# arpg/Kangaroo

Hardware: AMD Instinct MI355X
Metric: kinectfusion_frames_per_sec_640x480_to_512cubed_tsdf (higher is better)
Workload: dtype f32

## Files before the change

### include/kfx_extras.h

```cpp
#ifndef KFX_EXTRAS_H
#define KFX_EXTRAS_H

#include "kfx.h"

#ifdef __cplusplus
extern "C" {
#endif

int kfx_bilateral_guided_f32(const kfx_image* out, const kfx_image* in, const kfx_image* guide, float gs, float gr, float gc,
                             unsigned size, kfx_stream stream);
int kfx_bilateral_guided_u8(const kfx_image* out, const kfx_image* in, const kfx_image* guide, float gs, float gr, float gc,
                            unsigned size, kfx_stream stream);

int kfx_disp2depth(const kfx_image* in, const kfx_image* out, float fu, float baseline, float min_disp, kfx_stream stream);
int kfx_filter_bad_kinect_f32(const kfx_image* out, const kfx_image* in, kfx_stream stream);
int kfx_filter_bad_kinect_u16(const kfx_image* out, const kfx_image* in, kfx_stream stream);
int kfx_colour_vbo(const kfx_image* id, const kfx_image* vbo, const kfx_image* rgb, const float KT_cd[12], kfx_stream stream);

typedef struct kfx_keyframe {
    float K[4];
    float T_iw[12];
    kfx_image img;
} kfx_keyframe;
int kfx_texture_depth(const kfx_image* img, const kfx_keyframe* kfs, int n_kf, const kfx_image* depth, const kfx_image* norm,
                      const kfx_image* phong, const float T_wd[12], const float Kdepth[4], kfx_stream stream);

int kfx_raycast_box(const kfx_image* imgd, const float T_wc[12], const float K[4], const float boxmin[3], const float boxmax[3],
                    kfx_stream stream);
int kfx_raycast_sphere(const kfx_image* imgd, const kfx_image* img, const float T_wc[12], const float K[4], const float center[3],
                       float r, kfx_stream stream);
int kfx_raycast_plane(const kfx_image* imgd, const kfx_image* img, const float T_wc[12], const float K[4], const float n_w[3],
                      kfx_stream stream);
int kfx_sdf_distance(const kfx_image* dist, const kfx_image* depth, const kfx_volume* vol, const float T_wc[12], const float K[4],
                     float trunc_distance, kfx_stream stream);

#ifdef __cplusplus
}
#endif
#endif
```

### kangaroo_amd/_lib.py

```python
import ctypes as C
import os

_HERE = os.path.dirname(os.path.abspath(__file__))
LIB_PATH = os.environ.get("KFX_LIB_PATH") or os.path.join(_HERE, "libkfx.so")


class KfxImage(C.Structure):
    _fields_ = [("pitch", C.c_size_t), ("ptr", C.c_void_p), ("w", C.c_size_t), ("h", C.c_size_t)]


class KfxVolume(C.Structure):
    _fields_ = [("pitch", C.c_size_t), ("ptr", C.c_void_p), ("w", C.c_size_t), ("h", C.c_size_t),
                ("img_pitch", C.c_size_t), ("d", C.c_size_t),
                ("boxmin", C.c_float * 3), ("boxmax", C.c_float * 3)]


class KfxLss6(C.Structure):
    _fields_ = [("JTy", C.c_float * 6), ("JTJ", C.c_float * 21), ("sqErr", C.c_float), ("obs", C.c_uint)]


class KfxIcpLevel(C.Structure):
    _fields_ = [("Pl", KfxImage), ("Pr", KfxImage), ("Nr", KfxImage), ("K", C.c_float * 4), ("iterations", C.c_int), ("rotation_only", C.c_int)]


# ... 47 lines not shown
    "kfx_sdf_sphere": (C.c_int, [PV, PF, C.c_float, C.c_void_p]),
    "kfx_raycast_sdf_slab": (C.c_int, [C.c_void_p, C.c_int, PV, C.POINTER(KfxSlab), C.c_int, C.c_int, C.c_int, C.c_int, PF, PF,
                                       C.c_float, C.c_float, C.c_float, C.c_int, C.c_void_p]),
    "kfx_raycast_sdf_slab_h": (C.c_int, [C.c_void_p, C.c_int, PV, C.POINTER(KfxSlab), C.c_int, C.c_int, C.c_int, C.c_int, PF, PF,
                                       C.c_float, C.c_float, C.c_float, C.c_int, C.c_void_p]),
    "kfx_raycast_sdf_slab_tiles": (C.c_int, [C.c_void_p, C.c_void_p, C.c_size_t, C.c_int, C.c_int, C.c_int, C.c_int, C.c_void_p, C.c_int, C.c_void_p, C.c_void_p, C.c_int,
                                             PV, C.POINTER(KfxSlab), C.c_int, C.c_int, C.c_int, C.c_int, PF, PF, C.c_float, C.c_float, C.c_float, C.c_int, C.c_void_p]),
    "kfx_raycast_state_to_images": (C.c_int, [PI, PI, PI, C.c_void_p, C.c_void_p]),
    "kfx_sdf_fuse_color": (C.c_int, [PV, PV, PI, PI, PF, PF, PI, PF, PF, C.c_float, C.c_float, C.c_float, C.c_uint, C.c_void_p]),
    "kfx_raycast_sdf_color": (C.c_int, [PI, PI, PI, PV, PV, PF, PF, C.c_float, C.c_float, C.c_float, C.c_int, C.c_void_p]),
    "kfx_color_reset": (C.c_int, [PV, C.c_void_p]),
    "kfx_sdf_fuse_color_tracked": (C.c_int, [PV, PV, C.c_void_p, PI, PI, PF, PF, PI, PF, PF, C.c_float, C.c_float, C.c_float, C.c_uint, C.c_void_p]),
    "kfx_raycast_color_hits": (C.c_int, [C.c_int, C.POINTER(PI), C.POINTER(PI), PV, PF, PF, C.c_void_p]),
    "kfx_sdf_fuse_color_slab": (C.c_int, [PV, PV, C.POINTER(KfxSlab), PI, PI, PF, PF, PI, PF, PF, C.c_float, C.c_float, C.c_float, C.c_uint, C.c_void_p]),
    "kfx_raycast_sdf_slab_color": (C.c_int, [C.c_void_p, C.c_int, PV, PV, C.POINTER(KfxSlab), C.c_int, C.c_int, C.c_int, C.c_int, PF, PF,
                                             C.c_float, C.c_float, C.c_float, C.c_int, C.c_void_p]),
    "kfx_raycast_sdf_slab_tiles_color": (C.c_int, [C.c_void_p, C.c_void_p, C.c_size_t, C.c_int, C.c_int, C.c_int, C.c_int, C.c_void_p, C.c_int, C.c_void_p, C.c_void_p,
                                                   C.c_int, PV, PV, C.POINTER(KfxSlab), C.c_int, C.c_int, C.c_int, C.c_int, PF, PF, C.c_float, C.c_float, C.c_float,
                                                   C.c_int, C.c_void_p]),
    "kfx_slab_raycast_exact_tiled_color": (C.c_int, [PI, PI, PI, C.c_void_p, PV, PV, C.c_void_p, PF, PF, C.c_float, C.c_float, C.c_float, C.c_int, C.c_int,
                                                     C.c_void_p, C.c_void_p, C.POINTER(C.c_int), C.POINTER(C.c_int)]),
    "kfx_slab_frame_set_color": (C.c_int, [C.c_void_p, PV, PI, PF, PF]),
    "kfx_depth_to_vbo_normals_f32": (C.c_int, [PI, PI, PI, PF, C.c_float, C.c_void_p]),
    "kfx_depth_pyramid_vbo_normals_f32": (C.c_int, [PI, PI, PI, PF, C.c_int, C.c_float, C.c_void_p]),
    "kfx_bilateral_guided_f32": (C.c_int, [PI, PI, PI, C.c_float, C.c_float, C.c_float, C.c_uint, C.c_void_p]),
    "kfx_bilateral_guided_u8": (C.c_int, [PI, PI, PI, C.c_float, C.c_float, C.c_float, C.c_uint, C.c_void_p]),
    "kfx_texture_depth": (C.c_int, [PI, C.POINTER(KfxKeyframe), C.c_int, PI, PI, PI, PF, PF, C.c_void_p]),
    "kfx_disp2depth": (C.c_int, [PI, PI, C.c_float, C.c_float, C.c_float, C.c_void_p]),
    "kfx_filter_bad_kinect_f32": (C.c_int, [PI, PI, C.c_void_p]),
    "kfx_filter_bad_kinect_u16": (C.c_int, [PI, PI, C.c_void_p]),
    "kfx_colour_vbo": (C.c_int, [PI, PI, PI, PF, C.c_void_p]),
    "kfx_raycast_box": (C.c_int, [PI, PF, PF, PF, PF, C.c_void_p]),
    "kfx_raycast_sphere": (C.c_int, [PI, PI, PF, PF, PF, C.c_float, C.c_void_p]),
    "kfx_raycast_plane": (C.c_int, [PI, PI, PF, PF, PF, C.c_void_p]),
    "kfx_sdf_distance": (C.c_int, [PI, PI, PV, PF, PF, C.c_float, C.c_void_p]),
    "kfx_mc_count": (C.c_int, [PV, C.c_void_p, C.c_void_p]),
    "kfx_mc_emit": (C.c_int, [PV, PV, C.c_void_p, C.c_void_p, C.c_longlong, C.c_void_p, C.c_void_p, C.c_void_p, C.c_void_p]),
    "kfx_mesh_scratch_bytes": (C.c_size_t, [PV, C.c_int, C.POINTER(KfxSlab), C.c_int, C.c_int]),
    "kfx_mesh_plan": (C.c_int, [PV, C.c_int, C.POINTER(KfxSlab), C.c_int, C.c_int, C.c_void_p, C.c_size_t, C.POINTER(C.c_ulonglong), C.c_void_p]),
    "kfx_mesh_emit": (C.c_int, [PV, C.c_int, C.POINTER(KfxSlab), C.c_int, C.c_int, PV, C.c_void_p, C.c_size_t, C.POINTER(C.c_ulonglong), C.c_void_p,
                                C.c_void_p, C.c_void_p, C.c_void_p, C.c_void_p, C.c_void_p]),
    "kfx_icp_refine": (C.c_int, [C.POINTER(KfxIcpLevel), C.c_int, C.c_float, C.c_float, PI, PI, C.POINTER(C.c_double), PF,
                                 C.POINTER(C.c_uint), C.POINTER(C.c_int), C.c_void_p]),
    "kfx_pose_step": (C.c_int, [C.POINTER(C.c_double), C.POINTER(C.c_double), C.POINTER(C.c_double), PF]),
    "kfx_icp_refine_then": (C.c_int, [C.POINTER(KfxIcpLevel), C.c_int, C.c_float, C.c_float, PI, PI, C.POINTER(C.c_double), PF,
                                      C.POINTER(C.c_uint), C.POINTER(C.c_int), C.c_void_p, C.c_void_p, C.c_void_p]),
# ... 85 lines not shown
```

### kangaroo_amd/csrc/frame.hip

```cpp
#include <cmath>
#include <cstdlib>
#include <new>

#include "kfx_device.h"

struct kfx_frame {
    kfx_frame_config cfg;
    kfx_sdf_summary* summary;
    int track;
    long long frames;
    int slots;
    hipEvent_t* ev;
    long long* ev_frame;
    unsigned char* ev_mask;
    unsigned mask;
    kfx_image texels;
};

using namespace kfx;

static int valid_image(const kfx_image& im, size_t elem)
{
    return im.ptr && im.w > 0 && im.h > 0 && im.pitch >= im.w * elem;
}
// ... 128 lines not shown
    if (f->slots && f->mask) {
        const int slot = (int)(f->frames % f->slots);
        ev = f->ev + (size_t)slot * 4;
        m = f->mask;
        f->ev_frame[slot] = f->frames;
        f->ev_mask[slot] = (unsigned char)m;
    } else if (f->slots) {
        f->ev_frame[(int)(f->frames % f->slots)] = -1;
    }
    const hipStream_t s = (hipStream_t)stream;
    int e = 0;
    const auto record = [&](int k) {
        if (!(m & (1u << k))) return;
        const hipError_t he = hipEventRecord(ev[k], s);
        if (he != hipSuccess) {
            (void)hipGetLastError();
            f->ev_mask[(int)(f->frames % f->slots)] &= (unsigned char)~(1u << k);
            if (!e) e = set_error((int)he, "kfx_frame_step: hipEventRecord");
        }
    };
    record(0);
    const kfx_image* tex = ((parts & KFX_FRAME_PREPROCESS) && (parts & KFX_FRAME_FUSE) && f->texels.ptr) ? &f->texels : nullptr;
    if (!e && (parts & KFX_FRAME_PREPROCESS)) {
        e = kfx_bilateral_f32(&c.filtered, src, c.bilateral_gs, c.bilateral_gr, c.bilateral_size, c.bilateral_minval, 1, stream);
        if (!e) e = depth_to_vbo_normals_texels(&c.vbo, &c.normals, &c.filtered, c.K, 1.0f, tex, stream);
    }
    record(1);
    if (!e && (parts & KFX_FRAME_FUSE))
        e = sdf_fuse_texels(&c.vol, f->track ? f->summary : nullptr, &c.filtered, &c.normals, tex, T_cw, c.K, c.trunc_dist, c.max_w, c.mincostheta, c.fuse_flags, stream);
    record(2);
    if (!e && (parts & KFX_FRAME_RAYCAST)) {
        if (f->track) e = kfx_raycast_sdf_tracked(&c.ray_depth, &c.ray_norm, &c.ray_img, &c.vol, f->summary, T_wc, c.K, c.near, c.far, c.trunc_dist, 1, stream);
        else e = kfx_raycast_sdf(&c.ray_depth, &c.ray_norm, &c.ray_img, &c.vol, T_wc, c.K, c.near, c.far, c.trunc_dist, 1, stream);
    }
    record(3);
    f->frames += 1;
    return e;
}

extern "C" int kfx_frame_timings(kfx_frame* f, long long first_frame, int n_frames, float* ms)
{
    if (!f || !ms) return set_error(KFX_E_NULL, "kfx_frame_timings: null argument");
    if (!f->slots) return set_error(KFX_E_RANGE, "kfx_frame_timings: the frame was created without timing slots");
    if (n_frames <= 0) return 0;
    const long long last = first_frame + n_frames - 1;
    if (first_frame < 0 || last >= f->frames || f->frames - first_frame > f->slots) return set_error(KFX_E_RANGE, "kfx_frame_timings: frames not in the ring");
    const auto slot_of = [&](long long fr) { return (int)(fr % f->slots); };
    const auto first_event = [](unsigned m) { for (int k = 0; k < 4; ++k) if (m & (1u << k)) return k; return -1; };
// ... 43 lines not shown
```

### kangaroo_amd/csrc/preprocess.hip

```cpp

#include "kfx_device.h"
#include "host_args.h"

namespace kfx {

constexpr int BIL_MAX_R = 16;

struct BilParams {
    const unsigned char* in;
    size_t in_pitch;
    unsigned char* out;
    size_t out_pitch;
    int w, h;
    int iw, ih;
    int R;
    float gs, gr;
    float minval;
    int use_minval;
};

template <typename Ti>
__device__ __forceinline__ float load_clamped(const BilParams& p, int x, int y)
{
    x = min(max(x, 0), p.iw - 1);
    y = min(max(y, 0), p.ih - 1);
    return (float)reinterpret_cast<const Ti*>(p.in + (size_t)y * p.in_pitch)[x];
}

template <typename Ti, int TX, int TY, int PY>
__global__ __launch_bounds__(TX * TY) void k_bilateral(const BilParams p)
{
    extern __shared__ __attribute__((aligned(16))) float lds[];
    constexpr int NT = TX * TY;
    const int R = p.R, D = 2 * R + 1;
    const int TW = TX + 2 * R, TH = TY * PY + 2 * R;
    float* tile = lds;
    float* sw = lds + TW * TH;
    const int tid = threadIdx.x;
    const int bx = blockIdx.x * TX, by = blockIdx.y * (TY * PY);

    for (int i = tid; i < TW * TH; i += NT) {
        const int ty = i / TW, tx = i - ty * TW;
        tile[i] = load_clamped<Ti>(p, bx + tx - R, by + ty - R);
    }
    for (int i = tid; i < D * D; i += NT) {
        const int r = i / D - R, c = i % D - R;
        const float sd2 = (float)(r * r + c * c);
        sw[i] = __expf(-(sd2) / (2 * p.gs * p.gs));
    }
    __syncthreads();

    const int lx = tid % TX, ly0 = tid / TX;
    const int x = bx + lx;
    if (x >= p.w) return;
    const float inv2gr = 2 * p.gr * p.gr;
#pragma unroll
    for (int k = 0; k < PY; ++k) {
        const int ly = ly0 + k * TY;
        const int y = by + ly;
        if (y >= p.h) break;
        const float pc = tile[(ly + R) * TW + lx + R];
        float sum = 0.f, sumw = 0.f;
        if (!p.use_minval || pc >= p.minval) {
            for (int r = 0; r < D; ++r) {
                const float* trow = tile + (ly + r) * TW + lx;
                const float* srow = sw + r * D;
                for (int c = 0; c < D; ++c) {
                    const float q = trow[c];
                    if (!p.use_minval || q >= p.minval) {
                        const float id = pc - q;
                        const float id2 = id * id;
                        const float iw = __expf(-(id2) / inv2gr);
                        const float w = srow[c] * iw;
                        sumw += w;
                        sum += w * q;
                    }
                }
            }
        }
        reinterpret_cast<float*>(p.out + (size_t)y * p.out_pitch)[x] = sum / sumw;
    }
}

template <typename Ti, int R>
__global__ __launch_bounds__(256) void k_bilateral_fast(const BilParams p)
{
    constexpr int TX = 16, TY = 16, D = 2 * R + 1, TW = TX + 2 * R, TH = TY + 2 * R;
    __shared__ float tile[TH * TW];
    __shared__ float sw[D * D];
    const int tid = threadIdx.x;
    const int bx = blockIdx.x * TX, by = blockIdx.y * TY;
    for (int i = tid; i < TW * TH; i += 256) {
        const int ty = i / TW, tx = i - ty * TW;
        tile[i] = load_clamped<Ti>(p, bx + tx - R, by + ty - R);
    }
    if (tid < D * D) {
        const int r = tid / D - R, c = tid % D - R;
        sw[tid] = __expf(-((float)(r * r + c * c)) / (2 * p.gs * p.gs));
    }
    __syncthreads();
    const int lx = tid % TX, ly = tid / TX;
    const int x = bx + lx, y = by + ly;
    if (x >= p.w || y >= p.h) return;
    const float k = -1.0f / (2 * p.gr * p.gr);
    const float pc = tile[(ly + R) * TW + lx + R];
    const bool check = p.use_minval != 0;
    float sum = 0.f, sumw = 0.f;
#pragma unroll
    for (int r = 0; r < D; ++r)
#pragma unroll
        for (int c = 0; c < D; ++c) {
            const float q = tile[(ly + r) * TW + lx + c];
            const bool ok = !check || q >= p.minval;
            const float id = pc - q;
            const float w = sw[r * D + c] * __expf(id * id * k);
            sumw += ok ? w : 0.f;
            sum += ok ? w * q : 0.f;
        }
    if (check && !(pc >= p.minval)) sum = sumw = 0.f;
    reinterpret_cast<float*>(p.out + (size_t)y * p.out_pitch)[x] = sum / sumw;
}

template <typename Ti>
__global__ __launch_bounds__(256) void k_bilateral_global(const BilParams p)
{
    const int x = blockIdx.x * 64 + (threadIdx.x & 63), y = blockIdx.y * 4 + (threadIdx.x >> 6);
    if (x >= p.w || y >= p.h) return;
    const float pc = (float)reinterpret_cast<const Ti*>(p.in + (size_t)y * p.in_pitch)[x];
    float sum = 0.f, sumw = 0.f;
    if (!p.use_minval || pc >= p.minval) {
        for (int r = -p.R; r <= p.R; ++r)
            for (int c = -p.R; c <= p.R; ++c) {
                const float q = load_clamped<Ti>(p, x + c, y + r);
                if (!p.use_minval || q >= p.minval) {
                    const float sd2 = (float)(r * r + c * c);
                    const float id = pc - q;
                    const float id2 = id * id;
                    const float w = __expf(-(sd2) / (2 * p.gs * p.gs)) * __expf(-(id2) / (2 * p.gr * p.gr));
                    sumw += w;
                    sum += w * q;
                }
            }
    }
// ... 73 lines not shown
        const float4 Vc = r0[u], Vr = r0[u + 1], Vu = r1[u];
        const V3 a = v3(Vr.x - Vc.x, Vr.y - Vc.y, Vr.z - Vc.z);
        const V3 b = v3(Vu.x - Vc.x, Vu.y - Vc.y, Vu.z - Vc.z);
        const V3 axb = v3(a.y * b.z - a.z * b.y, a.z * b.x - a.x * b.z, a.x * b.y - a.y * b.x);
        const float mag = length(axb);
        N = make_float4(-axb.x / mag, -axb.y / mag, -axb.z / mag, 1.0f);
    }
    reinterpret_cast<float4*>(p.out + (size_t)v * p.out_pitch)[u] = N;
}

struct VboNrmParams {
    const unsigned char* in;
    size_t in_pitch;
    unsigned char *vbo, *nrm;
    size_t vpitch, npitch;
    int w, h;
    Intr K;
    float scale;
    unsigned char* tex;
    size_t tpitch;
    float* bmax;
    unsigned bw8;
};
__device__ __forceinline__ float4 vertex_of(const VboNrmParams& p, int u, int v)
{
    const float kz = p.scale * reinterpret_cast<const float*>(p.in + (size_t)v * p.in_pitch)[u];
    return make_float4(kz * ((float)u - p.K.u0) / p.K.fu, kz * ((float)v - p.K.v0) / p.K.fv, kz, 1.0f);
}
__global__ __launch_bounds__(256) void k_vbo_normals_f32(const VboNrmParams p)
{
    __shared__ float s_max[4][8];
    const int lane = threadIdx.x & 63, wv = threadIdx.x >> 6;
    const int u = blockIdx.x * 64 + lane, v = blockIdx.y * 4 + wv;
    float d = -__builtin_inff();
    if (u < p.w && v < p.h) {
        const float4 Vc = vertex_of(p, u, v);
        reinterpret_cast<float4*>(p.vbo + (size_t)v * p.vpitch)[u] = Vc;
        float4 N = make_float4(0.f, 0.f, 0.f, 0.f);
        if (u + 1 < p.w && v + 1 < p.h) {
            const float4 Vr = vertex_of(p, u + 1, v), Vu = vertex_of(p, u, v + 1);
            const V3 a = v3(Vr.x - Vc.x, Vr.y - Vc.y, Vr.z - Vc.z);
            const V3 b = v3(Vu.x - Vc.x, Vu.y - Vc.y, Vu.z - Vc.z);
            const V3 axb = v3(a.y * b.z - a.z * b.y, a.z * b.x - a.x * b.z, a.x * b.y - a.y * b.x);
            const float mag = length(axb);
            N = make_float4(-axb.x / mag, -axb.y / mag, -axb.z / mag, 1.0f);
        }
        reinterpret_cast<float4*>(p.nrm + (size_t)v * p.npitch)[u] = N;
        if (p.tex) {
            d = reinterpret_cast<const float*>(p.in + (size_t)v * p.in_pitch)[u];
            reinterpret_cast<float4*>(p.tex + (size_t)v * p.tpitch)[u] = make_float4(N.x, N.y, N.z, d);
        }
    }
    if (p.tex) {
        d = wave8_combine(fmaxf(d, -__builtin_inff()), [](float a, float b) { return fmaxf(a, b); });
        if ((lane & 7) == 0) s_max[wv][lane >> 3] = d;
        __syncthreads();
        if (threadIdx.x < 8)
            p.bmax[(size_t)blockIdx.y * p.bw8 + blockIdx.x * 8 + threadIdx.x] =
                fmaxf(fmaxf(s_max[0][threadIdx.x], s_max[1][threadIdx.x]), fmaxf(s_max[2][threadIdx.x], s_max[3][threadIdx.x]));
    }
}

struct EwParams {
    const unsigned char* in;
    size_t in_pitch;
    unsigned char* out;
    size_t out_pitch;
    int w, h;
    float s, offset;
};

__global__ __launch_bounds__(256) void k_scale_bias_f32(const EwParams p)
{
    const int x = blockIdx.x * 64 + (threadIdx.x & 63), y = blockIdx.y * 4 + (threadIdx.x >> 6);
    if (x >= p.w || y >= p.h) return;
    const float v1 = reinterpret_cast<const float*>(p.in + (size_t)y * p.in_pitch)[x];
    reinterpret_cast<float*>(p.out + (size_t)y * p.out_pitch)[x] = p.s * v1 + p.offset;
}

__global__ __launch_bounds__(256) void k_box_half_ignore_invalid_f32(const EwParams p)
{
    const int x = blockIdx.x * 64 + (threadIdx.x & 63), y = blockIdx.y * 4 + (threadIdx.x >> 6);
// ... 146 lines not shown
            const float ph = reinterpret_cast<const float*>(p.phong + (size_t)v * p.ppitch)[u];
            color = v3(ph, ph, ph);
        }
        const V3 c = div_s(color, w);
        out = make_float4(c.x, c.y, c.z, 1.f);
    }
    reinterpret_cast<float4*>(p.out + (size_t)v * p.opitch)[u] = out;
}

}

using namespace kfx;

static int check_image(const kfx_image* im, size_t elem, const char* what)
{
    if (!im || !im->ptr) return set_error(KFX_E_NULL, what);
    if (im->pitch < im->w * elem) return set_error(KFX_E_SHAPE, what);
    const size_t al = elem >= 16 ? 16 : elem;
    if (((uintptr_t)im->ptr | im->pitch) & (al - 1)) return set_error(KFX_E_ALIGN, what);
    if (im->w > (1u << 30) || im->h > (1u << 30)) return set_error(KFX_E_SHAPE, what);
    return 0;
}

template <typename Ti>
static int bilateral_launch(const kfx_image* out, const kfx_image* in, float gs, float gr, unsigned size,
                            float minval, int use_minval, kfx_stream stream)
{
    if (int e = check_image(out, 4, "BilateralFilter: output image")) return e;
    if (int e = check_image(in, sizeof(Ti), "BilateralFilter: input image")) return e;
    if (out->w == 0 || out->h == 0) return 0;
    if (in->w == 0 || in->h == 0) return set_error(KFX_E_SHAPE, "BilateralFilter: empty input");
    if (in->w < out->w || in->h < out->h) return set_error(KFX_E_SHAPE, "BilateralFilter: input smaller than output");
    if (size > 1024) return set_error(KFX_E_RANGE, "BilateralFilter: window radius");
    BilParams p;
    p.in = (const unsigned char*)in->ptr;
    p.in_pitch = in->pitch;
    p.out = (unsigned char*)out->ptr;
    p.out_pitch = out->pitch;
    p.w = (int)out->w;
    p.h = (int)out->h;
    p.iw = (int)in->w;
    p.ih = (int)in->h;
    p.R = (int)size;
    p.gs = gs;
    p.gr = gr;
    p.minval = minval;
    p.use_minval = use_minval;
    hipStream_t s = (hipStream_t)stream;
    if (math_mode() == KFX_MATH_FAST && p.R >= 1 && p.R <= 3) {
        dim3 grid(ceil_div(p.w, 16), ceil_div(p.h, 16));
        if (p.R == 3) hipLaunchKernelGGL((k_bilateral_fast<Ti, 3>), grid, dim3(256), 0, s, p);
        else if (p.R == 2) hipLaunchKernelGGL((k_bilateral_fast<Ti, 2>), grid, dim3(256), 0, s, p);
        else hipLaunchKernelGGL((k_bilateral_fast<Ti, 1>), grid, dim3(256), 0, s, p);
    } else if (p.R <= BIL_MAX_R) {
        const int D = 2 * p.R + 1;
        static const int shape = env_int("KFX_BILATERAL_TILE", 2);
#define KFX_BIL(TX_, TY_, PY_)                                                                                   \
    do {                                                                                                        \
        const size_t lds = (size_t)((TX_ + 2 * p.R) * (TY_ * PY_ + 2 * p.R) + D * D) * sizeof(float);           \
        dim3 grid(ceil_div(p.w, TX_), ceil_div(p.h, TY_ * PY_));                                                \
        hipLaunchKernelGGL((k_bilateral<Ti, TX_, TY_, PY_>), grid, dim3(TX_ * TY_), lds, s, p);                 \
    } while (0)
        switch (shape) {
        case 0: KFX_BIL(32, 8, 1); break;
        case 1: KFX_BIL(64, 4, 1); break;
        case 3: KFX_BIL(32, 8, 2); break;
        case 4: KFX_BIL(32, 8, 4); break;
        case 5: KFX_BIL(64, 4, 4); break;
        default: KFX_BIL(16, 16, 1); break;
        }
// ... 155 lines not shown
    hipLaunchKernelGGL(k_bilateral_guided<Tg>, dim3(ceil_div(g.b.w, 64), ceil_div(g.b.h, 4)), dim3(256), 0, (hipStream_t)stream, g);
    return check_launch("kfx_bilateral_guided");
}
extern "C" int kfx_bilateral_guided_f32(const kfx_image* out, const kfx_image* in, const kfx_image* guide, float gs, float gr, float gc,
                                        unsigned size, kfx_stream stream)
{
    return guided_launch<float>(out, in, guide, gs, gr, gc, size, stream);
}
extern "C" int kfx_bilateral_guided_u8(const kfx_image* out, const kfx_image* in, const kfx_image* guide, float gs, float gr, float gc,
                                       unsigned size, kfx_stream stream)
{
    return guided_launch<unsigned char>(out, in, guide, gs, gr, gc, size, stream);
}

namespace kfx {
int depth_to_vbo_normals_texels(const kfx_image* vbo, const kfx_image* nrm, const kfx_image* depth, const float K[4], float scale,
                                const kfx_image* texels, kfx_stream stream);
}
extern "C" int kfx_depth_to_vbo_normals_f32(const kfx_image* vbo, const kfx_image* nrm, const kfx_image* depth, const float K[4], float scale,
                                            kfx_stream stream)
{
    return kfx::depth_to_vbo_normals_texels(vbo, nrm, depth, K, scale, nullptr, stream);
}
int kfx::depth_to_vbo_normals_texels(const kfx_image* vbo, const kfx_image* nrm, const kfx_image* depth, const float K[4], float scale,
                                     const kfx_image* texels, kfx_stream stream)
{
    if (int e = check_image(vbo, 16, "DepthToVbo+Normals: vbo image")) return e;
    if (int e = check_image(nrm, 16, "DepthToVbo+Normals: normal image")) return e;
    if (int e = check_image(depth, 4, "DepthToVbo+Normals: depth image")) return e;
    if (!K) return set_error(KFX_E_NULL, "DepthToVbo+Normals: null intrinsics");
    if (vbo->w == 0 || vbo->h == 0) return 0;
    if (nrm->w != vbo->w || nrm->h != vbo->h || depth->w < vbo->w || depth->h < vbo->h)
        return set_error(KFX_E_SHAPE, "DepthToVbo+Normals: image sizes");
    const size_t tpitch = (vbo->w * 16 + 255) / 256 * 256;
    if (texels && (!texels->ptr || texels->w != vbo->w || texels->h != vbo->h || texels->pitch != tpitch || ((uintptr_t)texels->ptr & 15)))
        return set_error(KFX_E_SHAPE, "DepthToVbo+Normals: texel image");
    VboNrmParams p{(const unsigned char*)depth->ptr, depth->pitch, (unsigned char*)vbo->ptr, (unsigned char*)nrm->ptr, vbo->pitch, nrm->pitch,
                   (int)vbo->w, (int)vbo->h, Intr{K[0], K[1], K[2], K[3]}, scale, texels ? (unsigned char*)texels->ptr : nullptr, texels ? tpitch : 0,
                   texels ? reinterpret_cast<float*>((unsigned char*)texels->ptr + tpitch * vbo->h) : nullptr, (unsigned)((vbo->w + 63) / 64 * 8)};
    hipLaunchKernelGGL(k_vbo_normals_f32, dim3(ceil_div(p.w, 64), ceil_div(p.h, 4)), dim3(256), 0, (hipStream_t)stream, p);
    return check_launch("kfx_depth_to_vbo_normals_f32");
}

struct PyrParams {
    const unsigned char* d0;
    size_t d0_pitch;
    unsigned char* d[4];
    size_t dpitch[4];
    unsigned char *vbo[4], *nrm[4];
    size_t vpitch[4], npitch[4];
    int w[4], h[4];
    Intr K[4];
    int levels;
    float scale;
};
__device__ __forceinline__ float4 pyr_vertex(const Intr& K, float scale, float depth, int u, int v)
{
    const float kz = scale * depth;
    return make_float4(kz * ((float)u - K.u0) / K.fu, kz * ((float)v - K.v0) / K.fv, kz, 1.0f);
}
__global__ __launch_bounds__(256) void k_depth_pyramid_vbo_normals(const PyrParams p)
{
    constexpr int E0 = 40, E1 = 20, E2 = 10, E3 = 5;
    __shared__ float s0[E0 * E0], s1[E1 * E1], s2[E2 * E2], s3[E3 * E3];
    const int tid = threadIdx.x;
    {
        const int x0 = blockIdx.x * 32, y0 = blockIdx.y * 32;
        for (int t = tid; t < E0 * E0; t += 256) {
            const int ly = t / E0, lx = t - ly * E0, x = x0 + lx, y = y0 + ly;
            s0[t] = (x < p.w[0] && y < p.h[0]) ? reinterpret_cast<const float*>(p.d0 + (size_t)y * p.d0_pitch)[x] : 0.f;
        }
    }
    __syncthreads();
    float* const sl[4] = {s0, s1, s2, s3};
    const int ext[4] = {E0, E1, E2, E3};
#pragma unroll
    for (int l = 1; l < 4; ++l) {
        if (l < p.levels) {
            const int E = ext[l], Ef = ext[l - 1], S = 32 >> l;
            const int x0 = blockIdx.x * S, y0 = blockIdx.y * S;
            const float* f = sl[l - 1];
            for (int t = tid; t < E * E; t += 256) {
                const int ly = t / E, lx = t - ly * E;
// ... 2 lines not shown
                float sum = 0;
                if (isfinite(tx)) { sum += tx; n++; }
                if (isfinite(ty)) { sum += ty; n++; }
                if (isfinite(bx)) { sum += bx; n++; }
                if (isfinite(by)) { sum += by; n++; }
                const float m = n > 0 ? (sum / n) : __builtin_nanf("");
                sl[l][t] = m;
                const int x = x0 + lx, y = y0 + ly;
                if (lx < S && ly < S && x < p.w[l] && y < p.h[l]) reinterpret_cast<float*>(p.d[l] + (size_t)y * p.dpitch[l])[x] = m;
            }
        }
        __syncthreads();
    }
#pragma unroll
    for (int l = 0; l < 4; ++l) {
        if (l >= p.levels) break;
        const int E = ext[l], S = 32 >> l, w = p.w[l], h = p.h[l];
        const int x0 = blockIdx.x * S, y0 = blockIdx.y * S;
        const float* d = sl[l];
        const Intr K = p.K[l];
        for (int t = tid; t < S * S; t += 256) {
            const int ly = t / S, lx = t - ly * S, u = x0 + lx, v = y0 + ly;
            if (u >= w || v >= h) continue;
            const float4 Vc = pyr_vertex(K, p.scale, d[ly * E + lx], u, v);
            reinterpret_cast<float4*>(p.vbo[l] + (size_t)v * p.vpitch[l])[u] = Vc;
            float4 N = make_float4(0.f, 0.f, 0.f, 0.f);
            if (u + 1 < w && v + 1 < h) {
                const float4 Vr = pyr_vertex(K, p.scale, d[ly * E + lx + 1], u + 1, v), Vu = pyr_vertex(K, p.scale, d[(ly + 1) * E + lx], u, v + 1);
                const V3 a = v3(Vr.x - Vc.x, Vr.y - Vc.y, Vr.z - Vc.z);
                const V3 b = v3(Vu.x - Vc.x, Vu.y - Vc.y, Vu.z - Vc.z);
                const V3 axb = v3(a.y * b.z - a.z * b.y, a.z * b.x - a.x * b.z, a.x * b.y - a.y * b.x);
                const float mag = length(axb);
                N = make_float4(-axb.x / mag, -axb.y / mag, -axb.z / mag, 1.0f);
            }
            reinterpret_cast<float4*>(p.nrm[l] + (size_t)v * p.npitch[l])[u] = N;
        }
    }
}

extern "C" int kfx_depth_pyramid_vbo_normals_f32(const kfx_image* depth, const kfx_image* vbo, const kfx_image* nrm, const float* K, int levels,
                                                 float scale, kfx_stream stream)
{
    if (!depth || !vbo || !nrm || !K) return set_error(KFX_E_NULL, "DepthPyramidVboNormals: null argument");
    if (levels < 1 || levels > 4) return set_error(KFX_E_RANGE, "DepthPyramidVboNormals: 1 to 4 levels");
    PyrParams p;
    p.levels = levels;
    p.scale = scale;
    for (int l = 0; l < 4; ++l) {
        p.d[l] = p.vbo[l] = p.nrm[l] = nullptr;
        p.dpitch[l] = p.vpitch[l] = p.npitch[l] = 0;
        p.w[l] = p.h[l] = 0;
        p.K[l] = Intr{1.f, 1.f, 0.f, 0.f};
    }
    for (int l = 0; l < levels; ++l) {
        if (int e = check_image(&depth[l], 4, "DepthPyramidVboNormals: depth image")) return e;
        if (int e = check_image(&vbo[l], 16, "DepthPyramidVboNormals: vbo image")) return e;
// ... 56 lines not shown
```

### kangaroo_amd/csrc/slab_frame.hip

```cpp
#include <cmath>
#include <cstdlib>
#include <new>

#include "kfx_device.h"
#include "host_args.h"
#include "../../include/kfx_slab.h"
#include "slab_internal.h"

namespace {
constexpr int EV = 5;
constexpr int OPEN_SLOTS = 8;
constexpr int PIPE_MAX = KFX_SLAB_PIPE_MAX;
struct PendingFinal { long long frame; int set, os, slot, tiles; unsigned timing; };
}

struct kfx_slab_frame {
    kfx_slab_frame_config cfg;
    kfx_comm* comm;
    long long frames;
    void* exact;     size_t exact_bytes;
    void* strips;    size_t strips_bytes;
    void* keys;      size_t keys_bytes;
    void* bcast;     size_t bcast_bytes;
    int* h_open;
// ... 411 lines not shown
    if (f->slots) {
        slot = (int)(f->frames % f->slots);
        f->ev_frame[slot] = f->timing ? f->frames : -1;
        f->ev_mask[slot] = 0;
        if (f->timing) ev = f->ev + (size_t)slot * EV;
    }
    const auto record = [&](int k, hipStream_t on) {
        if (!ev || !(f->timing & (1u << k))) return;
        if (hipEventRecord(ev[k], on) == hipSuccess) f->ev_mask[slot] |= (unsigned char)(1u << k);
        else { (void)hipGetLastError(); note(set_error(KFX_E_RANGE, "kfx_slab_frame_step: hipEventRecord")); }
    };
    if (f->merge_pending && (parts & KFX_FRAME_RAYCAST)) {
        note(hip_status(hipStreamWaitEvent(s, f->merged, 0), "kfx_slab_frame_step: hipStreamWaitEvent"));
        f->merge_pending = 0;
    }
    note(check_open(f, false));

    record(0, s);
    const kfx_image* tex = ((parts & KFX_FRAME_PREPROCESS) && (parts & KFX_FRAME_FUSE) && f->texels.ptr &&
                            !(c.inputs == KFX_SLAB_INPUTS_BROADCAST && world > 1 && rank != 0)) ? &f->texels : nullptr;
    if (parts & KFX_FRAME_PREPROCESS) {
        const bool bcast = c.inputs == KFX_SLAB_INPUTS_BROADCAST && world > 1;
        if (!bcast || rank == 0) {
            note(kfx_bilateral_f32(&c.filtered, src, c.bilateral_gs, c.bilateral_gr, c.bilateral_size, c.bilateral_minval, 1, stream));
            note(kfx::depth_to_vbo_normals_texels(&c.vbo, &c.normals, &c.filtered, c.K, 1.0f, tex, stream));
        }
        if (bcast) note(kfx_slab_broadcast_inputs(&c.filtered, &c.normals, f->bcast, 0, comm, stream));
    }
    record(1, s);
    if (parts & KFX_FRAME_FUSE) {
        const bool own_only = c.halo == KFX_SLAB_HALO_EXCHANGE && world > 1;
        const size_t first = own_only ? L.z0 : L.s0, count = own_only ? L.z1 - L.z0 : L.s1 - L.s0;
        kfx_volume v = c.local;
        v.ptr = (unsigned char*)v.ptr + (first - L.s0) * v.img_pitch;
        v.d = count;
        const kfx_slab sl = {L.full_d, first, L.full_zmin, L.full_zmax};
        if (f->color) {
            kfx_volume cv = f->cvol;
            cv.ptr = (unsigned char*)cv.ptr + (first - L.s0) * cv.img_pitch;
            cv.d = count;
            float T_iw[12];
            for (int i = 0; i < 3; ++i)
                for (int j = 0; j < 4; ++j) {
                    float a = 0.f;
                    for (int k = 0; k < 3; ++k) a += f->T_cd[i * 4 + k] * T_cw[k * 4 + j];
                    T_iw[i * 4 + j] = j == 3 ? a + f->T_cd[i * 4 + 3] : a;
                }
            note(kfx_sdf_fuse_color_slab(&v, &cv, &sl, &c.filtered, &c.normals, T_cw, c.K, &f->rgb, T_iw, f->Kimg, c.trunc_dist, c.max_w, c.mincostheta,
// ... 134 lines not shown
```

### kangaroo_amd/roo.py

```python
import ctypes as C

import numpy as np
import torch

from . import _lib
from ._lib import KfxError, KfxImage, KfxVolume

_ELEM = {
    "f32": (np.float32, 1), "f32x4": (np.float32, 4), "u16": (np.uint16, 1), "u8": (np.uint8, 1),
    "u8x3": (np.uint8, 3),
    "u8x4": (np.uint8, 4),
}
PITCH_ALIGN = 256


def _stream(stream):
    if stream is not None:
        return C.c_void_p(int(stream))
    return C.c_void_p(torch.cuda.current_stream().cuda_stream)


def _fp(a, n):
    a = np.ascontiguousarray(np.asarray(a, dtype=np.float32).reshape(-1))
    if a.size != n:
# ... 655 lines not shown

def FilterBadKinectData(dFiltered, dKinectDepth, stream=None):
    L = _lib.load()
    fn = L.kfx_filter_bad_kinect_u16 if dKinectDepth.kind == "u16" else L.kfx_filter_bad_kinect_f32
    _lib.check(fn(dFiltered.ref(), dKinectDepth.ref(), _stream(stream)))


def ColourVbo(dId, dPd, dIc, KT_cd, stream=None):
    t, _t = _fp(KT_cd, 12)
    _lib.check(_lib.load().kfx_colour_vbo(dId.ref(), dPd.ref(), dIc.ref(), t, _stream(stream)))


def BilateralFilterGuided(dOut, dIn, dImg, gs, gr, gc, size, stream=None):
    L = _lib.load()
    fn = L.kfx_bilateral_guided_u8 if dImg.kind == "u8" else L.kfx_bilateral_guided_f32
    _lib.check(fn(dOut.ref(), dIn.ref(), dImg.ref(), gs, gr, gc, size, _stream(stream)))


def DepthToVboNormals(vbo, nrm, depth, K, scale=1.0, stream=None):
    k, _k = _fp(K, 4)
    _lib.check(_lib.load().kfx_depth_to_vbo_normals_f32(vbo.ref(), nrm.ref(), depth.ref(), k, scale, _stream(stream)))


def DepthPyramidVboNormals(depth, vbo, nrm, K_levels, scale=1.0, stream=None):
    n = 0
    while n < len(depth) and n < 4 and depth[n].w > 0 and depth[n].h > 0:
        n += 1
    if n == 0:
        return
    arrs = [(_lib.KfxImage * n)(*[im[l].view() for l in range(n)]) for im in (depth, vbo, nrm)]
    k, _k = _fp(np.concatenate([np.asarray(K_levels[l], np.float32).reshape(4) for l in range(n)]), 4 * n)
    _lib.check(_lib.load().kfx_depth_pyramid_vbo_normals_f32(arrs[0], arrs[1], arrs[2], k, n, scale, _stream(stream)))
    if len(depth) > n and n == 4 and depth[n].w > 0 and depth[n].h > 0:
        for l in range(n, len(depth)):
            if depth[l].w == 0 or depth[l].h == 0:
                break
            BoxHalfIgnoreInvalid(depth[l], depth[l - 1], stream)
            DepthToVboNormals(vbo[l], nrm[l], depth[l], K_levels[l], scale, stream)


def IcpRefine(kin_v, ray_v, ray_n, K_levels, its, icp_c, max_rmse, dWorkspace, dDebug=None, stream=None, before_wait=None):
    n = len(K_levels)
    order = list(range(n - 1, -1, -1))
    arr = (_lib.KfxIcpLevel * n)()
    for slot, l in enumerate(order):
        arr[slot].Pl, arr[slot].Pr, arr[slot].Nr = kin_v[l].view(), ray_v[l].view(), ray_n[l].view()
# ... 42 lines not shown
```

Measured before the change: 2470.

## Fuse bilateral filter with vertex/normal/texel generation into one frame-head kernel

Adds a k_frame_head kernel that bilateral-filters a tile plus a one-pixel halo into shared memory, then computes vertices, normals, texels and per-block depth maxima from the filtered values in the same launch. The frame and slab-frame pipelines call it in place of two separate kernels. This removes one launch and the global round trip of the filtered depth before normal computation. In exchange the halo pixels are filtered redundantly, the block carries 64 extra threads, and a fallback to the old path remains for unsupported sizes or overlapping buffers.

```diff
diff --git a/include/kfx_extras.h b/include/kfx_extras.h
--- a/include/kfx_extras.h
+++ b/include/kfx_extras.h
@@ -34,6 +34,11 @@
 int kfx_sdf_distance(const kfx_image* dist, const kfx_image* depth, const kfx_volume* vol, const float T_wc[12], const float K[4],
                      float trunc_distance, kfx_stream stream);
 
+int kfx_frame_head_f32(const kfx_image* filtered, const kfx_image* vbo, const kfx_image* nrm, const kfx_image* texels ,
+                       const kfx_image* raw, float gs, float gr, unsigned size, float minval, int use_minval, const float K[4], float scale,
+                       kfx_stream stream);
+size_t kfx_texel_image_bytes(size_t w, size_t h);
+
 #ifdef __cplusplus
 }
 #endif
diff --git a/kangaroo_amd/_lib.py b/kangaroo_amd/_lib.py
--- a/kangaroo_amd/_lib.py
+++ b/kangaroo_amd/_lib.py
@@ -93,6 +93,8 @@
                                                      C.c_void_p, C.c_void_p, C.POINTER(C.c_int), C.POINTER(C.c_int)]),
     "kfx_slab_frame_set_color": (C.c_int, [C.c_void_p, PV, PI, PF, PF]),
     "kfx_depth_to_vbo_normals_f32": (C.c_int, [PI, PI, PI, PF, C.c_float, C.c_void_p]),
+    "kfx_frame_head_f32": (C.c_int, [PI, PI, PI, PI, PI, C.c_float, C.c_float, C.c_uint, C.c_float, C.c_int, PF, C.c_float, C.c_void_p]),
+    "kfx_texel_image_bytes": (C.c_size_t, [C.c_size_t, C.c_size_t]),
     "kfx_depth_pyramid_vbo_normals_f32": (C.c_int, [PI, PI, PI, PF, C.c_int, C.c_float, C.c_void_p]),
     "kfx_bilateral_guided_f32": (C.c_int, [PI, PI, PI, C.c_float, C.c_float, C.c_float, C.c_uint, C.c_void_p]),
     "kfx_bilateral_guided_u8": (C.c_int, [PI, PI, PI, C.c_float, C.c_float, C.c_float, C.c_uint, C.c_void_p]),
diff --git a/kangaroo_amd/csrc/frame.hip b/kangaroo_amd/csrc/frame.hip
--- a/kangaroo_amd/csrc/frame.hip
+++ b/kangaroo_amd/csrc/frame.hip
@@ -174,8 +174,7 @@
     record(0);
     const kfx_image* tex = ((parts & KFX_FRAME_PREPROCESS) && (parts & KFX_FRAME_FUSE) && f->texels.ptr) ? &f->texels : nullptr;
     if (!e && (parts & KFX_FRAME_PREPROCESS)) {
-        e = kfx_bilateral_f32(&c.filtered, src, c.bilateral_gs, c.bilateral_gr, c.bilateral_size, c.bilateral_minval, 1, stream);
-        if (!e) e = depth_to_vbo_normals_texels(&c.vbo, &c.normals, &c.filtered, c.K, 1.0f, tex, stream);
+        e = kfx_frame_head_f32(&c.filtered, &c.vbo, &c.normals, tex, src, c.bilateral_gs, c.bilateral_gr, c.bilateral_size, c.bilateral_minval, 1, c.K, 1.0f, stream);
     }
     record(1);
     if (!e && (parts & KFX_FRAME_FUSE))
diff --git a/kangaroo_amd/csrc/preprocess.hip b/kangaroo_amd/csrc/preprocess.hip
--- a/kangaroo_amd/csrc/preprocess.hip
+++ b/kangaroo_amd/csrc/preprocess.hip
@@ -27,6 +27,57 @@
     return (float)reinterpret_cast<const Ti*>(p.in + (size_t)y * p.in_pitch)[x];
 }
 
+__device__ __forceinline__ float bil_spatial_weight(int i, int R, int D, float gs)
+{
+    const int r = i / D - R, c = i % D - R;
+    const float sd2 = (float)(r * r + c * c);
+    return __expf(-(sd2) / (2 * gs * gs));
+}
+__device__ __forceinline__ float bil_pixel_exact(const float* win, int TW, const float* sw, int D, float pc, float gr, float minval, int use_minval)
+{
+    const float inv2gr = 2 * gr * gr;
+    float sum = 0.f, sumw = 0.f;
+    if (!use_minval || pc >= minval) {
+        for (int r = 0; r < D; ++r) {
+            const float* trow = win + r * TW;
+            const float* srow = sw + r * D;
+            for (int c = 0; c < D; ++c) {
+                const float q = trow[c];
+                if (!use_minval || q >= minval) {
+                    const float id = pc - q;
+                    const float id2 = id * id;
+                    const float iw = __expf(-(id2) / inv2gr);
+                    const float w = srow[c] * iw;
+                    sumw += w;
+                    sum += w * q;
+                }
+            }
+        }
+    }
+    return sum / sumw;
+}
+template <int R>
+__device__ __forceinline__ float bil_pixel_fast(const float* win, int TW, const float* sw, float pc, float gr, float minval, int use_minval)
+{
+    constexpr int D = 2 * R + 1;
+    const float k = -1.0f / (2 * gr * gr);
+    const bool check = use_minval != 0;
+    float sum = 0.f, sumw = 0.f;
+#pragma unroll
+    for (int r = 0; r < D; ++r)
+#pragma unroll
+        for (int c = 0; c < D; ++c) {
+            const float q = win[r * TW + c];
+            const bool ok = !check || q >= minval;
+            const float id = pc - q;
+            const float w = sw[r * D + c] * __expf(id * id * k);
+            sumw += ok ? w : 0.f;
+            sum += ok ? w * q : 0.f;
+        }
+    if (check && !(pc >= minval)) sum = sumw = 0.f;
+    return sum / sumw;
+}
+
 template <typename Ti, int TX, int TY, int PY>
 __global__ __launch_bounds__(TX * TY) void k_bilateral(const BilParams p)
 {
@@ -43,42 +94,20 @@
         const int ty = i / TW, tx = i - ty * TW;
         tile[i] = load_clamped<Ti>(p, bx + tx - R, by + ty - R);
     }
-    for (int i = tid; i < D * D; i += NT) {
-        const int r = i / D - R, c = i % D - R;
-        const float sd2 = (float)(r * r + c * c);
-        sw[i] = __expf(-(sd2) / (2 * p.gs * p.gs));
-    }
+    for (int i = tid; i < D * D; i += NT) sw[i] = bil_spatial_weight(i, R, D, p.gs);
     __syncthreads();
 
     const int lx = tid % TX, ly0 = tid / TX;
     const int x = bx + lx;
     if (x >= p.w) return;
-    const float inv2gr = 2 * p.gr * p.gr;
 #pragma unroll
     for (int k = 0; k < PY; ++k) {
         const int ly = ly0 + k * TY;
         const int y = by + ly;
         if (y >= p.h) break;
         const float pc = tile[(ly + R) * TW + lx + R];
-        float sum = 0.f, sumw = 0.f;
-        if (!p.use_minval || pc >= p.minval) {
-            for (int r = 0; r < D; ++r) {
-                const float* trow = tile + (ly + r) * TW + lx;
-                const float* srow = sw + r * D;
-                for (int c = 0; c < D; ++c) {
-                    const float q = trow[c];
-                    if (!p.use_minval || q >= p.minval) {
-                        const float id = pc - q;
-                        const float id2 = id * id;
-                        const float iw = __expf(-(id2) / inv2gr);
-                        const float w = srow[c] * iw;
-                        sumw += w;
-                        sum += w * q;
-                    }
-                }
-            }
-        }
-        reinterpret_cast<float*>(p.out + (size_t)y * p.out_pitch)[x] = sum / sumw;
+        reinterpret_cast<float*>(p.out + (size_t)y * p.out_pitch)[x] =
+            bil_pixel_exact(tile + ly * TW + lx, TW, sw, D, pc, p.gr, p.minval, p.use_minval);
     }
 }
 
@@ -94,31 +123,14 @@
         const int ty = i / TW, tx = i - ty * TW;
         tile[i] = load_clamped<Ti>(p, bx + tx - R, by + ty - R);
     }
-    if (tid < D * D) {
-        const int r = tid / D - R, c = tid % D - R;
-        sw[tid] = __expf(-((float)(r * r + c * c)) / (2 * p.gs * p.gs));
-    }
+    if (tid < D * D) sw[tid] = bil_spatial_weight(tid, R, D, p.gs);
     __syncthreads();
     const int lx = tid % TX, ly = tid / TX;
     const int x = bx + lx, y = by + ly;
     if (x >= p.w || y >= p.h) return;
-    const float k = -1.0f / (2 * p.gr * p.gr);
     const float pc = tile[(ly + R) * TW + lx + R];
-    const bool check = p.use_minval != 0;
-    float sum = 0.f, sumw = 0.f;
-#pragma unroll
-    for (int r = 0; r < D; ++r)
-#pragma unroll
-        for (int c = 0; c < D; ++c) {
-            const float q = tile[(ly + r) * TW + lx + c];
-            const bool ok = !check || q >= p.minval;
-            const float id = pc - q;
-            const float w = sw[r * D + c] * __expf(id * id * k);
-            sumw += ok ? w : 0.f;
-            sum += ok ? w * q : 0.f;
-        }
-    if (check && !(pc >= p.minval)) sum = sumw = 0.f;
-    reinterpret_cast<float*>(p.out + (size_t)y * p.out_pitch)[x] = sum / sumw;
+    reinterpret_cast<float*>(p.out + (size_t)y * p.out_pitch)[x] =
+        bil_pixel_fast<R>(tile + ly * TW + lx, TW, sw, pc, p.gr, p.minval, p.use_minval);
 }
 
 template <typename Ti>
@@ -238,10 +250,22 @@
     float* bmax;
     unsigned bw8;
 };
+__device__ __forceinline__ float4 vertex_at(const Intr& K, float scale, float depth, int u, int v)
+{
+    const float kz = scale * depth;
+    return make_float4(kz * ((float)u - K.u0) / K.fu, kz * ((float)v - K.v0) / K.fv, kz, 1.0f);
+}
+__device__ __forceinline__ float4 normal_at(const float4 Vc, const float4 Vr, const float4 Vu)
+{
+    const V3 a = v3(Vr.x - Vc.x, Vr.y - Vc.y, Vr.z - Vc.z);
+    const V3 b = v3(Vu.x - Vc.x, Vu.y - Vc.y, Vu.z - Vc.z);
+    const V3 axb = v3(a.y * b.z - a.z * b.y, a.z * b.x - a.x * b.z, a.x * b.y - a.y * b.x);
+    const float mag = length(axb);
+    return make_float4(-axb.x / mag, -axb.y / mag, -axb.z / mag, 1.0f);
+}
 __device__ __forceinline__ float4 vertex_of(const VboNrmParams& p, int u, int v)
 {
-    const float kz = p.scale * reinterpret_cast<const float*>(p.in + (size_t)v * p.in_pitch)[u];
-    return make_float4(kz * ((float)u - p.K.u0) / p.K.fu, kz * ((float)v - p.K.v0) / p.K.fv, kz, 1.0f);
+    return vertex_at(p.K, p.scale, reinterpret_cast<const float*>(p.in + (size_t)v * p.in_pitch)[u], u, v);
 }
 __global__ __launch_bounds__(256) void k_vbo_normals_f32(const VboNrmParams p)
 {
@@ -255,11 +279,7 @@
         float4 N = make_float4(0.f, 0.f, 0.f, 0.f);
         if (u + 1 < p.w && v + 1 < p.h) {
             const float4 Vr = vertex_of(p, u + 1, v), Vu = vertex_of(p, u, v + 1);
-            const V3 a = v3(Vr.x - Vc.x, Vr.y - Vc.y, Vr.z - Vc.z);
-            const V3 b = v3(Vu.x - Vc.x, Vu.y - Vc.y, Vu.z - Vc.z);
-            const V3 axb = v3(a.y * b.z - a.z * b.y, a.z * b.x - a.x * b.z, a.x * b.y - a.y * b.x);
-            const float mag = length(axb);
-            N = make_float4(-axb.x / mag, -axb.y / mag, -axb.z / mag, 1.0f);
+            N = normal_at(Vc, Vr, Vu);
         }
         reinterpret_cast<float4*>(p.nrm + (size_t)v * p.npitch)[u] = N;
         if (p.tex) {
@@ -274,6 +294,86 @@
         if (threadIdx.x < 8)
             p.bmax[(size_t)blockIdx.y * p.bw8 + blockIdx.x * 8 + threadIdx.x] =
                 fmaxf(fmaxf(s_max[0][threadIdx.x], s_max[1][threadIdx.x]), fmaxf(s_max[2][threadIdx.x], s_max[3][threadIdx.x]));
+    }
+}
+
+struct FrameHeadParams {
+    BilParams b;
+    VboNrmParams v;
+    unsigned bh4;
+};
+constexpr int FH_TX = 32, FH_TY = 8, FH_NT = FH_TX * FH_TY + 64;
+template <bool FAST, int R>
+__global__ __launch_bounds__(FH_NT) void k_frame_head(const FrameHeadParams q)
+{
+    constexpr int TX = FH_TX, TY = FH_TY, NT = FH_NT, D = 2 * R + 1, TW = TX + 2 * R + 1, TH = TY + 2 * R + 1, FW = TX + 1;
+    __shared__ float tile[TH * TW];
+    __shared__ float sw[D * D];
+    __shared__ float filt[(TY + 1) * FW];
+    __shared__ float s_max[TY][TX / 8];
+    const BilParams& p = q.b;
+    const VboNrmParams& o = q.v;
+    const int tid = threadIdx.x;
+    const int bx = blockIdx.x * TX, by = blockIdx.y * TY;
+    {
+        constexpr int NL = (TW * TH + NT - 1) / NT;
+        float raw[NL];
+#pragma unroll
+        for (int k = 0; k < NL; ++k) {
+            const int i = tid + k * NT, ty = i / TW, tx = i - ty * TW;
+            raw[k] = i < TW * TH ? load_clamped<float>(p, bx + tx - R, by + ty - R) : 0.f;
+        }
+#pragma unroll
+        for (int k = 0; k < NL; ++k)
+            if (tid + k * NT < TW * TH) tile[tid + k * NT] = raw[k];
+    }
+    if (tid < D * D) sw[tid] = bil_spatial_weight(tid, R, D, p.gs);
+    __syncthreads();
+
+    const auto filter = [&](int fx, int fy, bool inside) {
+        if (bx + fx >= p.w || by + fy >= p.h) return;
+        const float* win = tile + fy * TW + fx;
+        const float pc = win[R * TW + R];
+        const float fd = FAST ? bil_pixel_fast<R>(win, TW, sw, pc, p.gr, p.minval, p.use_minval)
+                              : bil_pixel_exact(win, TW, sw, D, pc, p.gr, p.minval, p.use_minval);
+        filt[fy * FW + fx] = fd;
+        if (inside) reinterpret_cast<float*>(p.out + (size_t)(by + fy) * p.out_pitch)[bx + fx] = fd;
+    };
+    const bool own = tid < TX * TY;
+    const int lx = tid % TX, ly = tid / TX, x = bx + lx, y = by + ly;
+    if (own) filter(lx, ly, true);
+    const int a = tid - TX * TY;
+    if (a >= 0 && a < TY + TX) filter(a < TY ? TX : a - TY, a < TY ? a : TY, false);
+    __syncthreads();
+
+    float d = -__builtin_inff();
+    if (own && x < o.w && y < o.h) {
+        const int u = x, v = y;
+        const float dc = filt[ly * FW + lx];
+        const float4 Vc = vertex_at(o.K, o.scale, dc, u, v);
+        reinterpret_cast<float4*>(o.vbo + (size_t)v * o.vpitch)[u] = Vc;
+        float4 N = make_float4(0.f, 0.f, 0.f, 0.f);
+        if (u + 1 < o.w && v + 1 < o.h)
+            N = normal_at(Vc, vertex_at(o.K, o.scale, filt[ly * FW + lx + 1], u + 1, v), vertex_at(o.K, o.scale, filt[(ly + 1) * FW + lx], u, v + 1));
+        reinterpret_cast<float4*>(o.nrm + (size_t)v * o.npitch)[u] = N;
+        if (o.tex) {
+            d = dc;
+            reinterpret_cast<float4*>(o.tex + (size_t)v * o.tpitch)[u] = make_float4(N.x, N.y, N.z, d);
+        }
+    }
+    if (o.tex) {
+        if (own) {
+            d = wave8_combine(fmaxf(d, -__builtin_inff()), [](float m, float n) { return fmaxf(m, n); });
+            if ((tid & 7) == 0) s_max[ly][lx >> 3] = d;
+        }
+        __syncthreads();
+        const unsigned brow = blockIdx.y * (TY / 4) + ((tid >> 2) & 1), bcol = blockIdx.x * (TX / 8) + (tid & 3);
+        if (tid < 8 && brow < q.bh4) {
+            const int r = (tid >> 2) * 4, c = tid & 3;
+            o.bmax[(size_t)brow * o.bw8 + bcol] = fmaxf(fmaxf(s_max[r][c], s_max[r + 1][c]), fmaxf(s_max[r + 2][c], s_max[r + 3][c]));
+        } else if (tid >= 8 && tid < 16 && blockIdx.x == gridDim.x - 1 && brow < q.bh4 && bcol + TX / 8 < o.bw8) {
+            o.bmax[(size_t)brow * o.bw8 + bcol + TX / 8] = -__builtin_inff();
+        }
     }
 }
 
@@ -466,16 +566,19 @@
     return 0;
 }
 
-template <typename Ti>
-static int bilateral_launch(const kfx_image* out, const kfx_image* in, float gs, float gr, unsigned size,
-                            float minval, int use_minval, kfx_stream stream)
-{
+static int bilateral_args(const kfx_image* out, const kfx_image* in, size_t elem, unsigned size, bool& empty)
+{
+    empty = false;
     if (int e = check_image(out, 4, "BilateralFilter: output image")) return e;
-    if (int e = check_image(in, sizeof(Ti), "BilateralFilter: input image")) return e;
-    if (out->w == 0 || out->h == 0) return 0;
+    if (int e = check_image(in, elem, "BilateralFilter: input image")) return e;
+    if (out->w == 0 || out->h == 0) { empty = true; return 0; }
     if (in->w == 0 || in->h == 0) return set_error(KFX_E_SHAPE, "BilateralFilter: empty input");
     if (in->w < out->w || in->h < out->h) return set_error(KFX_E_SHAPE, "BilateralFilter: input smaller than output");
     if (size > 1024) return set_error(KFX_E_RANGE, "BilateralFilter: window radius");
+    return 0;
+}
+static BilParams bilateral_params(const kfx_image* out, const kfx_image* in, float gs, float gr, unsigned size, float minval, int use_minval)
+{
     BilParams p;
     p.in = (const unsigned char*)in->ptr;
     p.in_pitch = in->pitch;
@@ -490,6 +593,17 @@
     p.gr = gr;
     p.minval = minval;
     p.use_minval = use_minval;
+    return p;
+}
+
+template <typename Ti>
+static int bilateral_launch(const kfx_image* out, const kfx_image* in, float gs, float gr, unsigned size,
+                            float minval, int use_minval, kfx_stream stream)
+{
+    bool empty;
+    if (int e = bilateral_args(out, in, sizeof(Ti), size, empty)) return e;
+    if (empty) return 0;
+    const BilParams p = bilateral_params(out, in, gs, gr, size, minval, use_minval);
     hipStream_t s = (hipStream_t)stream;
     if (math_mode() == KFX_MATH_FAST && p.R >= 1 && p.R <= 3) {
         dim3 grid(ceil_div(p.w, 16), ceil_div(p.h, 16));
@@ -691,25 +805,74 @@
 {
     return kfx::depth_to_vbo_normals_texels(vbo, nrm, depth, K, scale, nullptr, stream);
 }
-int kfx::depth_to_vbo_normals_texels(const kfx_image* vbo, const kfx_image* nrm, const kfx_image* depth, const float K[4], float scale,
-                                     const kfx_image* texels, kfx_stream stream)
-{
+static int vbo_normals_args(const kfx_image* vbo, const kfx_image* nrm, const kfx_image* depth, const float K[4], const kfx_image* texels, bool& empty)
+{
+    empty = false;
     if (int e = check_image(vbo, 16, "DepthToVbo+Normals: vbo image")) return e;
     if (int e = check_image(nrm, 16, "DepthToVbo+Normals: normal image")) return e;
     if (int e = check_image(depth, 4, "DepthToVbo+Normals: depth image")) return e;
     if (!K) return set_error(KFX_E_NULL, "DepthToVbo+Normals: null intrinsics");
-    if (vbo->w == 0 || vbo->h == 0) return 0;
+    if (vbo->w == 0 || vbo->h == 0) { empty = true; return 0; }
     if (nrm->w != vbo->w || nrm->h != vbo->h || depth->w < vbo->w || depth->h < vbo->h)
         return set_error(KFX_E_SHAPE, "DepthToVbo+Normals: image sizes");
     const size_t tpitch = (vbo->w * 16 + 255) / 256 * 256;
     if (texels && (!texels->ptr || texels->w != vbo->w || texels->h != vbo->h || texels->pitch != tpitch || ((uintptr_t)texels->ptr & 15)))
         return set_error(KFX_E_SHAPE, "DepthToVbo+Normals: texel image");
-    VboNrmParams p{(const unsigned char*)depth->ptr, depth->pitch, (unsigned char*)vbo->ptr, (unsigned char*)nrm->ptr, vbo->pitch, nrm->pitch,
-                   (int)vbo->w, (int)vbo->h, Intr{K[0], K[1], K[2], K[3]}, scale, texels ? (unsigned char*)texels->ptr : nullptr, texels ? tpitch : 0,
-                   texels ? reinterpret_cast<float*>((unsigned char*)texels->ptr + tpitch * vbo->h) : nullptr, (unsigned)((vbo->w + 63) / 64 * 8)};
+    return 0;
+}
+static VboNrmParams vbo_normals_params(const kfx_image* vbo, const kfx_image* nrm, const kfx_image* depth, const float K[4], float scale, const kfx_image* texels)
+{
+    const size_t tpitch = (vbo->w * 16 + 255) / 256 * 256;
+    return VboNrmParams{(const unsigned char*)depth->ptr, depth->pitch, (unsigned char*)vbo->ptr, (unsigned char*)nrm->ptr, vbo->pitch, nrm->pitch,
+                        (int)vbo->w, (int)vbo->h, Intr{K[0], K[1], K[2], K[3]}, scale, texels ? (unsigned char*)texels->ptr : nullptr, texels ? tpitch : 0,
+                        texels ? reinterpret_cast<float*>((unsigned char*)texels->ptr + tpitch * vbo->h) : nullptr, (unsigned)((vbo->w + 63) / 64 * 8)};
+}
+int kfx::depth_to_vbo_normals_texels(const kfx_image* vbo, const kfx_image* nrm, const kfx_image* depth, const float K[4], float scale,
+                                     const kfx_image* texels, kfx_stream stream)
+{
+    bool empty;
+    if (int e = vbo_normals_args(vbo, nrm, depth, K, texels, empty)) return e;
+    if (empty) return 0;
+    const VboNrmParams p = vbo_normals_params(vbo, nrm, depth, K, scale, texels);
     hipLaunchKernelGGL(k_vbo_normals_f32, dim3(ceil_div(p.w, 64), ceil_div(p.h, 4)), dim3(256), 0, (hipStream_t)stream, p);
     return check_launch("kfx_depth_to_vbo_normals_f32");
 }
+
+static bool images_overlap(const kfx_image* a, size_t ea, const kfx_image* b, size_t eb)
+{
+    const uintptr_t a0 = (uintptr_t)a->ptr, a1 = a0 + a->pitch * (a->h - 1) + a->w * ea;
+    const uintptr_t b0 = (uintptr_t)b->ptr, b1 = b0 + b->pitch * (b->h - 1) + b->w * eb;
+    return a0 < b1 && b0 < a1;
+}
+extern "C" int kfx_frame_head_f32(const kfx_image* filtered, const kfx_image* vbo, const kfx_image* nrm, const kfx_image* texels, const kfx_image* raw,
+                                  float gs, float gr, unsigned size, float minval, int use_minval, const float K[4], float scale, kfx_stream stream)
+{
+    bool no_filter, no_maps;
+    if (int e = bilateral_args(filtered, raw, 4, size, no_filter)) return e;
+    if (int e = vbo_normals_args(vbo, nrm, filtered, K, texels, no_maps)) return e;
+    static const int enabled = env_int("KFX_FRAME_HEAD", 1);
+    if (!enabled || no_filter || no_maps || size < 1 || size > 3 || filtered->w != vbo->w || filtered->h != vbo->h || images_overlap(raw, 4, filtered, 4)) {
+        if (int e = kfx_bilateral_f32(filtered, raw, gs, gr, size, minval, use_minval, stream)) return e;
+        return kfx::depth_to_vbo_normals_texels(vbo, nrm, filtered, K, scale, texels, stream);
+    }
+    FrameHeadParams q{bilateral_params(filtered, raw, gs, gr, size, minval, use_minval ? 1 : 0), vbo_normals_params(vbo, nrm, filtered, K, scale, texels),
+                      (unsigned)((vbo->h + 3) / 4)};
+    const dim3 grid(ceil_div(q.b.w, FH_TX), ceil_div(q.b.h, FH_TY));
+    const hipStream_t s = (hipStream_t)stream;
+    const bool fast = math_mode() == KFX_MATH_FAST;
+#define KFX_FH(R_)                                                                                   \
+    do {                                                                                             \
+        if (fast) hipLaunchKernelGGL((k_frame_head<true, R_>), grid, dim3(FH_NT), 0, s, q);          \
+        else hipLaunchKernelGGL((k_frame_head<false, R_>), grid, dim3(FH_NT), 0, s, q);              \
+    } while (0)
+    if (size == 3) KFX_FH(3);
+    else if (size == 2) KFX_FH(2);
+    else KFX_FH(1);
+#undef KFX_FH
+    return check_launch("kfx_frame_head_f32");
+}
+
+extern "C" size_t kfx_texel_image_bytes(size_t w, size_t h) { return kfx::texel_image_bytes(w, h); }
 
 struct PyrParams {
     const unsigned char* d0;
@@ -723,11 +886,6 @@
     int levels;
     float scale;
 };
-__device__ __forceinline__ float4 pyr_vertex(const Intr& K, float scale, float depth, int u, int v)
-{
-    const float kz = scale * depth;
-    return make_float4(kz * ((float)u - K.u0) / K.fu, kz * ((float)v - K.v0) / K.fv, kz, 1.0f);
-}
 __global__ __launch_bounds__(256) void k_depth_pyramid_vbo_normals(const PyrParams p)
 {
     constexpr int E0 = 40, E1 = 20, E2 = 10, E3 = 5;
@@ -776,16 +934,12 @@
         for (int t = tid; t < S * S; t += 256) {
             const int ly = t / S, lx = t - ly * S, u = x0 + lx, v = y0 + ly;
             if (u >= w || v >= h) continue;
-            const float4 Vc = pyr_vertex(K, p.scale, d[ly * E + lx], u, v);
+            const float4 Vc = vertex_at(K, p.scale, d[ly * E + lx], u, v);
             reinterpret_cast<float4*>(p.vbo[l] + (size_t)v * p.vpitch[l])[u] = Vc;
             float4 N = make_float4(0.f, 0.f, 0.f, 0.f);
             if (u + 1 < w && v + 1 < h) {
-                const float4 Vr = pyr_vertex(K, p.scale, d[ly * E + lx + 1], u + 1, v), Vu = pyr_vertex(K, p.scale, d[(ly + 1) * E + lx], u, v + 1);
-                const V3 a = v3(Vr.x - Vc.x, Vr.y - Vc.y, Vr.z - Vc.z);
-                const V3 b = v3(Vu.x - Vc.x, Vu.y - Vc.y, Vu.z - Vc.z);
-                const V3 axb = v3(a.y * b.z - a.z * b.y, a.z * b.x - a.x * b.z, a.x * b.y - a.y * b.x);
-                const float mag = length(axb);
-                N = make_float4(-axb.x / mag, -axb.y / mag, -axb.z / mag, 1.0f);
+                const float4 Vr = vertex_at(K, p.scale, d[ly * E + lx + 1], u + 1, v), Vu = vertex_at(K, p.scale, d[(ly + 1) * E + lx], u, v + 1);
+                N = normal_at(Vc, Vr, Vu);
             }
             reinterpret_cast<float4*>(p.nrm[l] + (size_t)v * p.npitch[l])[u] = N;
         }
diff --git a/kangaroo_amd/csrc/slab_frame.hip b/kangaroo_amd/csrc/slab_frame.hip
--- a/kangaroo_amd/csrc/slab_frame.hip
+++ b/kangaroo_amd/csrc/slab_frame.hip
@@ -457,8 +457,7 @@
     if (parts & KFX_FRAME_PREPROCESS) {
         const bool bcast = c.inputs == KFX_SLAB_INPUTS_BROADCAST && world > 1;
         if (!bcast || rank == 0) {
-            note(kfx_bilateral_f32(&c.filtered, src, c.bilateral_gs, c.bilateral_gr, c.bilateral_size, c.bilateral_minval, 1, stream));
-            note(kfx::depth_to_vbo_normals_texels(&c.vbo, &c.normals, &c.filtered, c.K, 1.0f, tex, stream));
+            note(kfx_frame_head_f32(&c.filtered, &c.vbo, &c.normals, tex, src, c.bilateral_gs, c.bilateral_gr, c.bilateral_size, c.bilateral_minval, 1, c.K, 1.0f, stream));
         }
         if (bcast) note(kfx_slab_broadcast_inputs(&c.filtered, &c.normals, f->bcast, 0, comm, stream));
     }
diff --git a/kangaroo_amd/roo.py b/kangaroo_amd/roo.py
--- a/kangaroo_amd/roo.py
+++ b/kangaroo_amd/roo.py
@@ -701,6 +701,15 @@
     _lib.check(_lib.load().kfx_depth_to_vbo_normals_f32(vbo.ref(), nrm.ref(), depth.ref(), k, scale, _stream(stream)))
 
 
+def FrameHead(filtered, vbo, nrm, raw, gs, gr, size, K, minval=None, scale=1.0, texels=None, stream=None):
+    k, _k = _fp(K, 4)
+    tex = None
+    if texels is not None:
+        tex = C.byref(KfxImage((vbo.w * 16 + 255) // 256 * 256, texels.data_ptr(), vbo.w, vbo.h))
+    _lib.check(_lib.load().kfx_frame_head_f32(filtered.ref(), vbo.ref(), nrm.ref(), tex, raw.ref(), gs, gr, size,
+                                              0.0 if minval is None else minval, 0 if minval is None else 1, k, scale, _stream(stream)))
+
+
 def DepthPyramidVboNormals(depth, vbo, nrm, K_levels, scale=1.0, stream=None):
     n = 0
     while n < len(depth) and n < 4 and depth[n].w > 0 and depth[n].h > 0:
```

Measured after the change: 2470. About the same (-0.0%).
